# JARVIS-MoCap/JARVIS-HybridNet

Measured on AMD Instinct MI355X. Metric: multi-view frames/s (12cam 1280x1024, 23kpt, 64^3 grid), higher is better.
Workload: dtype f32; 1 GPU; BASELINE configs[2]: HybridNet 12-camera 1280x1024, 23 kpts, 64^3 grid, small/small; cameras=12, joints=23, grid=64, streams=3, parallelism=single GPU, 3 time batches in flight on 3 HIP streams, hipgraph=False

## Files before the change

### include/jarvis_hip.h

```cpp
#ifndef JARVIS_HIP_H
#define JARVIS_HIP_H
#include <stdint.h>

#ifdef __cplusplus
extern "C" {
#endif

#define JH_ABI_VERSION 4

const char* jh_last_error(void);
int jh_abi_version(void);

#define JH_PRECISION_DEFAULT (-1)
#define JH_PRECISION_F32 0
#define JH_PRECISION_BF16X3 1
#define JH_PRECISION_BF16X3_WIDE 2
int jh_set_precision(int mode);
int jh_get_precision(void);

typedef struct jh_params jh_params;
int jh_params_create(jh_params** out);
int jh_params_set(jh_params* p, const char* key, const float* host, int64_t numel);
void jh_params_destroy(jh_params* p);

// ... 258 lines not shown
int jh_predictor2d_forward_sensor(jh_predictor2d* pr, const uint8_t* frames_dev, const jh_sensor_surface* surface,
                                  int32_t* points_dev, float* conf_dev, int32_t* valid_dev, void* stream);

int jh_predictor2d_forward_images(jh_predictor2d* pr, const void* const* images_host, int n_images, int format,
                                  const jh_yuv_surface* yuv, const jh_sensor_surface* sensor,
                                  int32_t* points_dev, float* conf_dev, int32_t* valid_dev, void* stream);

int jh_profile_begin(void);
int jh_profile_end(int* n_records);
int jh_profile_get(int i, char* name, int name_cap, double* ms, double* flops, double* bytes);

int jh_op_conv(int nd, int kind, int k, int stride, int pad, int cin, int cout,
               const float* w_host, const float* b_host, const float* x_dev, int n, int d, int h,
               int w, const float* gate_dev, int norm_act, float* y_dev, void* stream);
long jh_deconv4_window_launches(void);
int jh_conv_form(int nd, int kind, int k, int stride, int pad, int cin, int cout, int has_bias,
                 int want_stats, int gate , int precision,
                 int in_px , char* name, int name_cap);
int jh_node_form(int c, int cout, int n, int h, int w, int n_in, const int* modes, int act, int batch_class,
                 int want_pool, char* name, int name_cap, int32_t out[8]);
typedef struct jh_op_operand {
  const double* in_sums_host;
  int32_t in_act;
  int32_t latency_class;
  int32_t want_stats;
  int32_t se_c, se_s;
  float se_inv_hw;
  const float *se_wr_host, *se_br_host, *se_we_host, *se_be_host;
  const double* se_pool_host;
} jh_op_operand;
int jh_op_conv_operand(int nd, int kind, int k, int stride, int pad, int cin, int cout,
                       const float* w_host, const float* b_host, const float* x_dev, int n, int d, int h,
                       int w, const float* gate_dev, const jh_op_operand* operand, float* y_dev, void* stream);
int jh_op_se_gate(const double* pool_host, int n, int c, int squeeze, float inv_hw, const float* wr_host,
                  const float* br_host, const float* we_host, const float* be_host, float* gate_dev, void* stream);
int jh_op_norm_apply(const float* x_dev, int n, int c, int d, int h, int w, const double* sums_host, int act,
                     const float* r1_dev, const double* r1_sums_host, const float* r2_dev, int write_y, int want_pool,
                     int min_block_kb, float* y_dev, double* pool_host, void* stream);
int jh_op_depthwise(int k, int c, const float* w_host, const float* x_dev, int n, int h, int w,
                    int norm_act, float* y_dev, void* stream);
int jh_op_depthwise_pool(int k, int c, const float* w_host, const float* x_dev, int n, int h, int w,
                         float* y_dev, float* pool_dev, void* stream);

int jh_op_yuv420_to_bgr(const uint8_t* frames_dev, int format, int n, int h, int w, uint8_t* out_bgr_dev,
                        void* stream);
int jh_op_yuv_surface_to_bgr(const uint8_t* frames_dev, const jh_yuv_surface* surface, int n, int h, int w,
                             uint8_t* out_bgr_dev, void* stream);
int jh_op_sensor_to_bgr(const uint8_t* frames_dev, const jh_sensor_surface* surface, int n, int h, int w,
                        uint8_t* out_bgr_dev, void* stream);

int64_t jh_joint_argmax_all_workspace_bytes(int n, int hh, int wh, int jp);
int jh_op_joint_argmax_all(const float* heat_dev, int n, int hh, int wh, int j, int jp, int32_t* idx_dev,
                           float* max_dev, void* workspace_dev, int64_t workspace_bytes, void* stream);

int jh_op_bifpn_node(int n_in, const int* modes, const float* weights, int act, int n, int c, int cout,
                     int h, int w, const float* x0_dev, const float* x1_dev, const float* x2_dev,
                     const float* dw_host, const float* pw_host, const float* bias_host, float* y_dev,
                     void* stream);
typedef struct jh_op_node_ex {
  int32_t batch_class;
  int32_t want_pool;
  const double* in_sums_host[3];
  int64_t in_count[3];
  float* y_pool_dev;
  int32_t* pool_written_host;
  double* out_sums_host;
// ... 11 lines not shown
```

### jarvis-hybridnet_amd/_native.py

```python
import ctypes
import math
import os
from typing import NamedTuple

import torch

_HERE = os.path.dirname(os.path.abspath(__file__))
LIB_PATH = os.environ.get("JH_LIBRARY_PATH") or os.path.join(_HERE, "libjarvis_hip.so")
_lib = None

c_void_p, c_int, c_float, c_int64 = ctypes.c_void_p, ctypes.c_int, ctypes.c_float, ctypes.c_int64
c_char_p = ctypes.c_char_p


class PredictorConfig(ctypes.Structure):
    _fields_ = [("num_cameras", ctypes.c_int32), ("num_joints", ctypes.c_int32),
                ("center_size", ctypes.c_int32), ("bbox", ctypes.c_int32),
                ("roi_cube_size", c_float), ("grid_spacing", c_float),
                ("center_model", ctypes.c_int32), ("kp_model", ctypes.c_int32),
                ("img_h", ctypes.c_int32), ("img_w", ctypes.c_int32),
                ("time_batch", ctypes.c_int32), ("time_batch_3d", ctypes.c_int32),
                ("cam_lo", ctypes.c_int32),
                ("cam_n", ctypes.c_int32), ("mean", c_float * 3), ("std", c_float * 3),
                ("precision", ctypes.c_int32)]
# ... 185 lines not shown
    "jh_op_joint_peaks_refine": (c_int, [c_void_p, c_int, c_int, c_int, c_int, c_void_p, c_int, c_int, c_void_p,
                                         c_void_p]),
    "jh_op_triangulate_joints": (c_int, [c_void_p, c_int, c_int, c_int, c_void_p, c_void_p, c_void_p, c_int,
                                         ctypes.POINTER(Joints3dParamsStruct), c_void_p, c_void_p, c_void_p, c_void_p,
                                         c_void_p]),
    "jh_predictor_triangulate_joints": (c_int, [c_void_p, c_void_p, c_int, c_void_p,
                                                ctypes.POINTER(Joints3dParamsStruct)] + [c_void_p] * 6),
    "jh_predictor_set_joint_mask": (c_int, [c_void_p, c_int, c_void_p, ctypes.POINTER(Joints3dParamsStruct), c_void_p]),
    "jh_predictor_get_joint_mask": (c_int, [c_void_p, c_void_p, c_void_p, c_void_p]),
    "jh_predictor_stage_3d_joint_masked": (c_int, [c_void_p, c_void_p, c_int] + [c_void_p] * 6),
    "jh_reproject_joint_masked_workspace_bytes": (c_int64, [c_int, c_int, c_int, c_int]),
    "jh_reproject_forward_joint_masked": (c_int, [c_void_p, c_int, c_int, c_int, c_void_p, c_void_p, c_void_p,
                                                  c_void_p, c_void_p, c_int, c_float, c_void_p, c_void_p, c_void_p,
                                                  c_void_p, c_int64, c_void_p]),
    "jh_joint_argmax_all_workspace_bytes": (c_int64, [c_int, c_int, c_int, c_int]),
    "jh_op_joint_argmax_all": (c_int, [c_void_p, c_int, c_int, c_int, c_int, c_int, c_void_p, c_void_p, c_void_p,
                                       c_int64, c_void_p]),
    "jh_predictor2d_create": (c_int, [c_void_p, c_void_p, ctypes.POINTER(PredictorConfig),
                                      ctypes.POINTER(c_void_p)]),
    "jh_predictor2d_destroy": (None, [c_void_p]),
    "jh_predictor2d_forward": (c_int, [c_void_p] * 6),
    "jh_predictor2d_forward_u8": (c_int, [c_void_p] * 6),
    "jh_predictor2d_forward_yuv": (c_int, [c_void_p, c_void_p, c_int, c_void_p, c_void_p, c_void_p, c_void_p]),
    "jh_predictor_debug": (c_int, [c_void_p, c_void_p, c_void_p, c_void_p, c_void_p, c_void_p]),
    "jh_predictor_hybridnet_forward": (c_int, [c_void_p] * 9),
    "jh_op_conv": (c_int, [c_int] * 7 + [c_void_p, c_void_p, c_void_p] + [c_int] * 4 +
                   [c_void_p, c_int, c_void_p, c_void_p]),
    "jh_deconv4_window_launches": (ctypes.c_long, []),
    "jh_conv_form": (c_int, [c_int] * 12 + [c_char_p, c_int]),
    "jh_node_form": (c_int, [c_int] * 6 + [ctypes.POINTER(c_int)] + [c_int] * 3 +
                     [c_char_p, c_int, ctypes.POINTER(ctypes.c_int32)]),
    "jh_op_conv_operand": (c_int, [c_int] * 7 + [c_void_p, c_void_p, c_void_p] + [c_int] * 4 +
                           [c_void_p, ctypes.POINTER(OpOperand), c_void_p, c_void_p]),
    "jh_op_se_gate": (c_int, [c_void_p, c_int, c_int, c_int, c_float] + [c_void_p] * 6),
    "jh_op_norm_apply": (c_int, [c_void_p] + [c_int] * 5 + [c_void_p, c_int, c_void_p, c_void_p, c_void_p, c_int,
                                                           c_int, c_int, c_void_p, c_void_p, c_void_p]),
    "jh_op_depthwise": (c_int, [c_int, c_int, c_void_p, c_void_p, c_int, c_int, c_int, c_int,
                                c_void_p, c_void_p]),
    "jh_op_depthwise_pool": (c_int, [c_int, c_int, c_void_p, c_void_p, c_int, c_int, c_int, c_void_p, c_void_p,
                                     c_void_p]),
    "jh_op_yuv420_to_bgr": (c_int, [c_void_p, c_int, c_int, c_int, c_int, c_void_p, c_void_p]),
    "jh_op_bifpn_node": (c_int, [c_int, ctypes.POINTER(c_int), ctypes.POINTER(c_float), c_int, c_int, c_int,
                                 c_int, c_int, c_int, c_void_p, c_void_p, c_void_p, c_void_p, c_void_p,
                                 c_void_p, c_void_p, c_void_p]),
    "jh_op_bifpn_node_ex": (c_int, [c_int, ctypes.POINTER(c_int), ctypes.POINTER(c_float), c_int, c_int, c_int,
                                    c_int, c_int, c_int, c_void_p, c_void_p, c_void_p, c_void_p, c_void_p,
                                    c_void_p, c_void_p, ctypes.POINTER(OpNodeEx), c_void_p]),
}


def symbols():
    return sorted(_SIGS)


def lib():
    global _lib
    if _lib is None:
        if not os.path.isfile(LIB_PATH):
            raise RuntimeError(
                "jarvis_hybridnet_amd: %s is missing -- build it with "
                "`python -c 'import __graft_entry__ as g; g.build()'` (hipcc, gfx950). "
                "There is no CPU fallback." % LIB_PATH)
        handle = ctypes.CDLL(LIB_PATH)
        for name, (res, args) in _SIGS.items():
            fn = getattr(handle, name)
            fn.restype, fn.argtypes = res, args
# ... 398 lines not shown
```

### jarvis-hybridnet_amd/csrc/api.hip

```cpp
#include <cstring>
#include <memory>
#include "../../include/jarvis_hip.h"
#include <cstdlib>
#include "nets.h"
#include "bifpn_node.h"
#include "views2d.h"
#include "subjects.h"
#include "joints3d.h"
#include "tracks.h"

namespace jh {
static thread_local std::string g_err;
void set_error(const std::string& msg) { g_err = msg; }
}

using namespace jh;

struct jh_params { ParamMap map; };
struct jh_efftrack { EffTrackPlan plan; };
struct jh_v2v { V2VPlan plan; };

namespace {

struct Scratch {
// ... 1683 lines not shown
                        (int32_t)ch.lds, ch.pool ? 1 : 0};
  std::copy(v, v + 8, out);
  return 0;
}

static int op_upload_stats(Scratch& sc, const double* sums_host, int n, int c, int Cp, double** dev) {
  std::vector<double> st((size_t)n * Cp * kStatW, 0.0);
  for (int b = 0; b < n; ++b)
    for (int ch = 0; ch < c; ++ch) {
      st[((size_t)b * Cp + ch) * kStatW] = sums_host[((size_t)b * c + ch) * 2];
      st[((size_t)b * Cp + ch) * kStatW + kLimbs] = sums_host[((size_t)b * c + ch) * 2 + 1];
    }
  return op_upload(sc, st.data(), st.size(), dev);
}

static int op_upload_se(Scratch& sc, const double* pool_host, int n, int C, int Cp, int S, float inv_hw,
                        const float* wr, const float* br, const float* we, const float* be, SeGate* out) {
  JH_REQUIRE(pool_host && wr && br && we && be && C >= 1 && C <= Cp && S >= 1, "squeeze-excite recipe");
  std::vector<double> pl((size_t)n * Cp * kLimbs, 0.0);
  for (int b = 0; b < n; ++b)
    for (int ch = 0; ch < C; ++ch) pl[((size_t)b * Cp + ch) * kLimbs] = pool_host[(size_t)b * C + ch];
  double* pool = nullptr;
  float *dwr = nullptr, *dbr = nullptr, *dwe = nullptr, *dbe = nullptr;
  if (op_upload(sc, pl.data(), pl.size(), &pool) || op_upload(sc, wr, (size_t)S * C, &dwr) ||
      op_upload(sc, br, (size_t)S, &dbr) || op_upload(sc, we, (size_t)C * S, &dwe) || op_upload(sc, be, (size_t)C, &dbe))
    return 1;
  out->pool = pool; out->wr = dwr; out->br = dbr; out->we = dwe; out->be = dbe;
  out->C = C; out->S = S; out->inv_hw = inv_hw;
  return 0;
}

static int op_conv_body(int nd, int kind, int k, int stride, int pad, int cin, int cout, const float* w_host,
                        const float* b_host, const float* x_dev, int n, int d, int h, int w, const float* gate_dev,
                        int norm_act, const jh_op_operand* opd, float* y_dev, hipStream_t s, const char* who) {
  const bool recipe = opd && opd->se_pool_host;
  const bool want_stats = opd ? opd->want_stats != 0 : norm_act >= 0;
  const bool plain_out = !want_stats && !gate_dev && !recipe;
  const ConvDesc desc = kind == 0 ? conv_desc(nd, k, stride, pad, cin, cout)
                                  : (kind == 1 ? deconv2d_k4s2p1_desc(cin, cout) : deconv3d_k2s2_desc(cin, cout));
  Scratch sc;
  Act x, y;
  if (nd == 2) d = 1;
  if (sc.act(n, d, h, w, cin, &x)) return 1;
  int Do, Ho, Wo;
  conv_out_shape(desc, d, h, w, &Do, &Ho, &Wo);
  if (sc.act(n, Do, Ho, Wo, cout, &y)) return 1;
  JH_CHECK_HIP(hipMemsetAsync(y.p, kind == 1 && plain_out ? 0xFF : 0, y.bytes(), s));
  ConvUse use;
  use.desc = desc; use.desc.latency_class = opd ? opd->latency_class : 0;
  use.transposed = kind != 0; use.has_bias = b_host != nullptr; use.want_stats = want_stats;
  use.gate = recipe ? ConvGate::Recipe : (gate_dev ? ConvGate::Tensor : ConvGate::None);
  use.precision = precision_mode();
  use.in_px = x.Cp;
  ConvLayer layer;
  if (make_conv_layer(use, w_host, b_host, y.D, y.H, y.W, &layer)) return 1;
  double* stats = nullptr;
  float* gate_p = nullptr;
  if (want_stats) {
    if (sc.get(reinterpret_cast<void**>(&stats), (size_t)n * y.Cp * kStatW * sizeof(double))) return 1;
    JH_CHECK_HIP(hipMemsetAsync(stats, 0, (size_t)n * y.Cp * kStatW * sizeof(double), s));
  }
  if (gate_dev) {
    if (sc.get(reinterpret_cast<void**>(&gate_p), (size_t)n * x.Cp * sizeof(float))) return 1;
    JH_CHECK_HIP(hipMemsetAsync(gate_p, 0, (size_t)n * x.Cp * sizeof(float), s));
    JH_CHECK_HIP(hipMemcpy2DAsync(gate_p, x.Cp * sizeof(float), gate_dev, cin * sizeof(float), cin * sizeof(float), n,
                                  hipMemcpyDeviceToDevice, s));
  }
  InNorm in;
  SeGate se;
  if (opd && opd->in_sums_host) {
    double* st = nullptr;
    if (op_upload_stats(sc, opd->in_sums_host, n, cin, x.Cp, &st)) return 1;
    in.stats = st; in.inv = 1.f / (float)x.pixels(); in.act = opd->in_act;
  }
  if (recipe) {
    JH_REQUIRE(opd->se_c == cin, "the gate recipe has one gate per input channel");
    if (op_upload_se(sc, opd->se_pool_host, n, opd->se_c, x.Cp, opd->se_s, opd->se_inv_hw, opd->se_wr_host,
                     opd->se_br_host, opd->se_we_host, opd->se_be_host, &se)) return 1;
  }
  if (launch_to_channel_last(x_dev, x, s)) return 1;
  if (layer.launch(x, y, gate_p, stats, in, recipe ? &se : nullptr, s)) return 1;
  if (!opd && norm_act >= 0 && launch_norm_apply(y, stats, norm_act, nullptr, nullptr, y.p, nullptr, s)) return 1;
  if (launch_from_channel_last(y, y_dev, s)) return 1;
  if (hipStreamSynchronize(s) != hipSuccess) { set_error(std::string("stream sync failed in ") + who); return 1; }
  return 0;
}

int jh_op_conv(int nd, int kind, int k, int stride, int pad, int cin, int cout,
               const float* w_host, const float* b_host, const float* x_dev, int n, int d, int h,
               int w, const float* gate_dev, int norm_act, float* y_dev, void* stream) {
  return op_conv_body(nd, kind, k, stride, pad, cin, cout, w_host, b_host, x_dev, n, d, h, w, gate_dev, norm_act,
                      nullptr, y_dev, static_cast<hipStream_t>(stream), "jh_op_conv");
}

int jh_op_conv_operand(int nd, int kind, int k, int stride, int pad, int cin, int cout,
                       const float* w_host, const float* b_host, const float* x_dev, int n, int d, int h,
                       int w, const float* gate_dev, const jh_op_operand* operand, float* y_dev, void* stream) {
  JH_REQUIRE(operand && w_host && x_dev && y_dev && n >= 1, "bad argument");
  JH_REQUIRE(operand->in_act >= ACT_NONE && operand->in_act <= ACT_SILU, "jh_op_conv_operand: in_act");
  JH_REQUIRE(operand->latency_class == 0 || operand->latency_class == 1, "jh_op_conv_operand: latency_class");
  JH_REQUIRE(!(gate_dev && operand->se_pool_host), "either a gate tensor or a gate recipe");
  return op_conv_body(nd, kind, k, stride, pad, cin, cout, w_host, b_host, x_dev, n, d, h, w, gate_dev, -1, operand,
                      y_dev, static_cast<hipStream_t>(stream), "jh_op_conv_operand");
}

int jh_op_se_gate(const double* pool_host, int n, int c, int squeeze, float inv_hw, const float* wr_host,
                  const float* br_host, const float* we_host, const float* be_host, float* gate_dev, void* stream) {
  hipStream_t s = static_cast<hipStream_t>(stream);
  JH_REQUIRE(gate_dev && n >= 1, "bad argument");
  Scratch sc;
  SeGate se;
  const int Cp = cpad(c);
  if (op_upload_se(sc, pool_host, n, c, Cp, squeeze, inv_hw, wr_host, br_host, we_host, be_host, &se)) return 1;
  float* gate = nullptr;
  if (sc.get(reinterpret_cast<void**>(&gate), (size_t)n * Cp * sizeof(float))) return 1;
  if (launch_se_gate(se.pool, n, c, Cp, squeeze, inv_hw, se.wr, se.br, se.we, se.be, gate, s)) return 1;
  JH_CHECK_HIP(hipMemcpy2DAsync(gate_dev, c * sizeof(float), gate, Cp * sizeof(float), c * sizeof(float), n,
                                hipMemcpyDeviceToDevice, s));
  JH_CHECK_HIP(hipStreamSynchronize(s));
  return 0;
}

int jh_op_norm_apply(const float* x_dev, int n, int c, int d, int h, int w, const double* sums_host, int act,
                     const float* r1_dev, const double* r1_sums_host, const float* r2_dev, int write_y, int want_pool,
                     int min_block_kb, float* y_dev, double* pool_host, void* stream) {
  hipStream_t s = static_cast<hipStream_t>(stream);
  JH_REQUIRE(x_dev && sums_host && n >= 1 && (!write_y || y_dev) && (!want_pool || pool_host), "bad argument");
  Scratch sc;
  Act x, r1, r2;
  if (sc.act(n, d, h, w, c, &x) || launch_to_channel_last(x_dev, x, s)) return 1;
  if (r1_dev && (sc.act(n, d, h, w, c, &r1) || launch_to_channel_last(r1_dev, r1, s))) return 1;
  if (r2_dev && (sc.act(n, d, h, w, c, &r2) || launch_to_channel_last(r2_dev, r2, s))) return 1;
  double *st = nullptr, *st1 = nullptr, *pool = nullptr;
  if (op_upload_stats(sc, sums_host, n, c, x.Cp, &st)) return 1;
  if (r1_sums_host && op_upload_stats(sc, r1_sums_host, n, c, x.Cp, &st1)) return 1;
  const size_t npl = (size_t)n * x.Cp * kLimbs;
// ... 259 lines not shown
```

### jarvis-hybridnet_amd/csrc/conv3d_wino.hip

```cpp
#include <vector>
#include "conv_mfma.h"
#include "conv3d_wino.h"

namespace jh {

constexpr int kWSV = 12;

constexpr int kWTZ = 4;
template <int NR, bool SH = false>
__global__ __launch_bounds__(256, 1) void conv3d_wino_kernel(const WinoArgs a) {
  constexpr int kWPZ = kWTZ + 2;
  constexpr int kWNP = kWPZ * (SH ? 108 : kWPY * kWPX);
  extern __shared__ __attribute__((aligned(16))) float lds_all[];
  const int nrm_floats = a.in_stats ? 2 * a.cin_p : 0;
  float* nrm = lds_all;
  float* R = lds_all + nrm_floats;
  float* V = R + kWNP * 8;
  float* X = R;
  const int tid = threadIdx.x;
  const int lane = tid & 63;
  const int wave = __builtin_amdgcn_readfirstlane(tid >> 6);
  const int mrow = lane & 15, kq = lane >> 4;

  const BlockId bid = xcd_block();
// ... 213 lines not shown
        X[(wave * NR * 16 + nr * 16 + mrow) * 2 + 1] = t2;
      }
    }
    __syncthreads();
    if (tid < NR * 16) {
      const int ch = nb0 * 16 + tid;
      if (ch < a.cout_p) {
        float t1 = 0.f, t2 = 0.f;
#pragma unroll
        for (int w = 0; w < 4; ++w) {
          t1 += X[(w * NR * 16 + tid) * 2 + 0];
          t2 += X[(w * NR * 16 + tid) * 2 + 1];
        }
        stat_add(a.stats + ((size_t)n * a.cout_p + ch) * kStatW, t1, t2);
      }
    }
  }
}

template <int NR, bool SH = false>
static int launch_wino_nr(const WinoArgs& a, dim3 grid, size_t lds, hipStream_t s) {
  auto kern = conv3d_wino_kernel<NR, SH>;
  static bool big = false;
  if (!big) {
    JH_CHECK_HIP(hipFuncSetAttribute(reinterpret_cast<const void*>(kern),
                                     hipFuncAttributeMaxDynamicSharedMemorySize, 160 * 1024));
    big = true;
  }
  hipLaunchKernelGGL(kern, grid, dim3(256), lds, s, a);
  JH_CHECK_HIP(hipGetLastError());
  return 0;
}

int pack_wino_weights(int cin, int cout, const float* w, const float* b, ConvWeights* out) {
  const int cin_p = cpad(cin), cout_p16 = round_up(cout, 16);
  const int nk8 = cin_p / 8, nb = cout_p16 / 16;
  static const float G[4][3] = {{1.f, 0.f, 0.f}, {.5f, .5f, .5f}, {.5f, -.5f, .5f}, {0.f, 0.f, 1.f}};
  std::vector<float> packed((size_t)16 * 3 * nk8 * nb * 128, 0.f);
  for (int co = 0; co < cout; ++co)
    for (int ci = 0; ci < cin; ++ci)
      for (int dz = 0; dz < 3; ++dz) {
        const float* g = w + (((size_t)co * cin + ci) * 3 + dz) * 9;
        double tmp[4][3];
        for (int fy = 0; fy < 4; ++fy)
          for (int kx = 0; kx < 3; ++kx) {
            double s = 0.0;
            for (int ky = 0; ky < 3; ++ky) s += (double)G[fy][ky] * g[ky * 3 + kx];
            tmp[fy][kx] = s;
          }
        const int k8 = ci / 8, kq = (ci % 8) / 2, j = ci % 2;
        const int nbk = co / 16, nn = co % 16;
        const int lane = kq * 16 + nn;
        for (int fy = 0; fy < 4; ++fy)
          for (int fx = 0; fx < 4; ++fx) {
            double s = 0.0;
            for (int kx = 0; kx < 3; ++kx) s += tmp[fy][kx] * (double)G[fx][kx];
            const int f = fy * 4 + fx;
            packed[((((size_t)f * 3 + dz) * nk8 + k8) * nb + nbk) * 128 + lane * 2 + j] = (float)s;
          }
      }
  out->cin_p = cin_p; out->cout_p16 = cout_p16; out->phase_stride = packed.size();
  return upload_conv_weights(packed.data(), packed.size() * sizeof(float), b, cout, out);
}

std::vector<int> wino_tables(int D, int H, int W, int cin_p) {
  const WinoTiling g = wino_tiling(D, H, W, 4);
  std::vector<int> t;
  if (!g.shaped) return t;
  t.assign((size_t)3 * kWinoShapeWords, 0);
  const int rz = D % 4 ? D % 4 : 4;
  for (int lc = 1; lc <= 3; ++lc) {
    const int PW = (2 << lc) + 2, PH = (32 >> lc) + 2, TH = 32 >> lc, TW = 2 << lc;
    const int hy = H - (lc == 3 ? g.H44 : 0), wx = W - (lc == 1 ? g.W44 : 0);
    const int ry = hy % TH ? hy % TH : TH, rx = wx % TW ? wx % TW : TW;
    int* tab = t.data() + (size_t)(lc - 1) * kWinoShapeWords;
    for (int lane = 0; lane < 64; ++lane) {
      unsigned m[7] = {0, 0, 0, 0, 0, 0, 0};
      for (int it = 0; it < kWinoShapeIter; ++it) {
        const int idx = lane + it * 64, pix = idx >> 1, q = lane & 1;
        const int px = pix % PW, py = (pix / PW) % PH, pz = pix / (PW * PH);
        tab[it * 64 + lane] = (((pz * H + py) * W + px) * cin_p + q * 4) * 4;
        m[0] |= (unsigned)(pz == 0) << it; m[1] |= (unsigned)(pz > rz) << it;
        m[2] |= (unsigned)(py == 0) << it; m[3] |= (unsigned)(py > ry) << it;
        m[4] |= (unsigned)(px == 0) << it; m[5] |= (unsigned)(px > rx) << it;
        m[6] |= (unsigned)(idx >= 6 * PW * PH * 2) << it;
      }
      for (int k = 0; k < 7; ++k) tab[(kWinoShapeIter + k) * 64 + lane] = (int)m[k];
    }
  }
  return t;
}
// ... 39 lines not shown
```

### jarvis-hybridnet_amd/csrc/conv_layer.h

```cpp
#pragma once
#include <string>
#include <vector>
#include "jh_common.h"

namespace jh {

enum class ConvForm {
  Mfma,
  Wino,
  WinoBf16x3,
  ConvBf16x3,
  Deconv4Bf16x3,
  DeconvC1,
};

enum class ConvGate { None = 0, Tensor = 1, Recipe = 2 };

struct ConvUse {
  ConvDesc desc;
  bool transposed = false;
  bool has_bias = false;
  bool want_stats = false;
  ConvGate gate = ConvGate::None;
  int precision = 0;
  int in_px = 0;
};

struct ConvChoice {
  ConvForm form = ConvForm::Mfma;
  WeightLayout layout = WeightLayout::Plain;
  int wino_variant = 0;
};
ConvChoice choose_conv(const ConvUse& u);
std::string conv_choice_name(const ConvChoice& c);

std::vector<float> taps_major(const float* w, int channels, int taps, int Cp);

struct ConvLayer {
  ConvLayer() = default;
  ConvLayer(const ConvLayer&) = delete;
  ConvLayer& operator=(const ConvLayer&) = delete;
  ~ConvLayer();

  ConvChoice choice;
  ConvDesc desc{};
  ConvWeights w;
  int* wino_tiles = nullptr;
  size_t table_bytes = 0;

  int launch(const Act& x, const Act& y, const float* gate, double* stats, const InNorm& in, const SeGate* se,
             hipStream_t s) const;
  std::string profile_name(int out_w) const;
  size_t device_bytes() const { return w.phase_stride * desc.nphase * sizeof(float) + table_bytes; }
};

int make_conv_layer(const ConvUse& u, const float* w_host, const float* b_host, int D, int H, int W, ConvLayer* out);

}
// ... 1 lines not shown
```

### jarvis-hybridnet_amd/csrc/conv_layer.hip

```cpp
#include <cstdlib>
#include "conv_layer.h"
#include "conv_mfma.h"
#include "conv3d_wino.h"

namespace jh {

static int knob_now(const char* name, int unset) {
  const char* e = getenv(name);
  return e ? atoi(e) : unset;
}

static WeightLayout conv_weight_layout(const ConvUse& u) {
  const ConvDesc& d = u.desc;
  const int cin_p = cpad(d.cin), cout_p = cpad(d.cout), cout_p16 = round_up(d.cout, 16);
  if (d.nd == 3 && d.k == 3 && d.stride == 2 && d.ostride == 1) return WeightLayout::TapPaired;
  if (d.nd == 2 && d.ostride > 1) {
    const int wmode = knob_now("JH_DECONV4_WINDOW", 1);
    if (!u.want_stats && u.gate == ConvGate::None && wmode != 0 && deconv4_window_eligible(cin_p, cout_p, wmode >= 2))
      return WeightLayout::Window;
    if (deconv4_eligible(cin_p, cout_p16)) return WeightLayout::ChannelPaired;
  }
  return WeightLayout::Plain;
}

ConvChoice choose_conv(const ConvUse& u) {
  const ConvDesc& d = u.desc;
  const bool ungated = u.gate == ConvGate::None;
  const bool bare_deconv2d = d.nd == 2 && d.ostride > 1 && u.transposed && !u.has_bias && !u.want_stats && ungated;
  const int in_px = u.in_px ? u.in_px : cpad(d.cin);
  const auto form = [](ConvForm f, int wino_variant = 0) { return ConvChoice{f, WeightLayout::Plain, wino_variant}; };
  if (bare_deconv2d && d.cout == 1) return form(ConvForm::DeconvC1);
  if (d.nd == 3 && d.k == 3 && d.stride == 1 && d.ostride == 1 && d.phase[0].pad[2] == 1 && !u.transposed && ungated &&
      knob_now("JH_WINO", 1) != 0)
    return form(u.precision >= 1 ? ConvForm::WinoBf16x3 : ConvForm::Wino, knob_now("JH_WINO_PW", 1) != 0 ? 4 : 0);
  if (bare_deconv2d && u.precision >= 1 && deconv4_bf16x3_eligible(d.cout)) return form(ConvForm::Deconv4Bf16x3);
  if (!u.transposed && ungated && conv_bf16x3_eligible(d) && in_px == cpad(d.cin) &&
      (u.precision == 2 || (u.precision == 1 && d.nd == 3)))
    return form(ConvForm::ConvBf16x3);
  return ConvChoice{ConvForm::Mfma, conv_weight_layout(u), 0};
}

std::string conv_choice_name(const ConvChoice& c) {
  static const char* const forms[] = {"mfma", "wino", "wino_bf16x3", "conv_bf16x3", "deconv4_bf16x3", "deconv_c1"};
  static const char* const layouts[] = {"", "_paired", "_tappair", "_window"};
  return std::string(forms[(int)c.form]) + (c.form == ConvForm::Mfma ? layouts[(int)c.layout] : "");
}

std::vector<float> taps_major(const float* w, int channels, int taps, int Cp) {
  std::vector<float> wt((size_t)taps * Cp, 0.f);
  for (int c = 0; c < channels; ++c)
    for (int t = 0; t < taps; ++t) wt[(size_t)t * Cp + c] = w[(size_t)c * taps + t];
  return wt;
}

ConvLayer::~ConvLayer() {
  free_conv_weights(&w);
  if (wino_tiles) (void)hipFree(wino_tiles);
}

int make_conv_layer(const ConvUse& u, const float* w_host, const float* b_host, int D, int H, int W, ConvLayer* out) {
  const ConvDesc& d = u.desc;
  JH_REQUIRE(w_host && (b_host != nullptr) == u.has_bias, "conv layer weights / bias");
  const ConvChoice c = out->choice = choose_conv(u);
  const int in_px = u.in_px ? u.in_px : cpad(d.cin);
  out->desc = d;
  switch (c.form) {
    case ConvForm::DeconvC1: {
      const std::vector<float> wt = taps_major(w_host, d.cin, 16, in_px);
      out->w.phase_stride = wt.size() / d.nphase;
      return upload_conv_weights(wt.data(), wt.size() * sizeof(float), nullptr, 0, &out->w);
    }
    case ConvForm::ConvBf16x3: return pack_conv_bf16x3_weights(d, w_host, b_host, &out->w);
    case ConvForm::Deconv4Bf16x3: return pack_deconv4_bf16x3_weights(d.cin, d.cout, w_host, &out->w);
    case ConvForm::WinoBf16x3: return pack_bf16x3_weights(d.cin, d.cout, w_host, b_host, &out->w);
    case ConvForm::Mfma: return pack_conv_weights(d, w_host, b_host, u.transposed, c.layout, &out->w);
    case ConvForm::Wino: break;
  }
  if (pack_wino_weights(d.cin, d.cout, w_host, b_host, &out->w)) return 1;
  const std::vector<int> tt = wino_tables(D, H, W, in_px);
  if (tt.empty()) return 0;
  out->table_bytes = tt.size() * sizeof(int);
  JH_CHECK_HIP(hipMalloc(&out->wino_tiles, out->table_bytes));
  JH_CHECK_HIP(hipMemcpy(out->wino_tiles, tt.data(), out->table_bytes, hipMemcpyHostToDevice));
  return 0;
}

int ConvLayer::launch(const Act& x, const Act& y, const float* gate, double* stats, const InNorm& in, const SeGate* se,
                      hipStream_t s) const {
  JH_REQUIRE(choice.form == ConvForm::Mfma || (!gate && !(se && se->pool)), "only the MFMA form takes a gate");
  switch (choice.form) {
    case ConvForm::DeconvC1: return launch_deconv_c1(x, in.stats, in.inv, in.act, w.w, y, s);
    case ConvForm::ConvBf16x3: return launch_conv_bf16x3(desc, w, x, y, stats, s, &in);
    case ConvForm::Deconv4Bf16x3: return launch_deconv4_bf16x3(w, x, y, s, &in);
    case ConvForm::WinoBf16x3: return launch_conv3d_bf16x3(w, x, y, stats, s, &in);
    case ConvForm::Wino: return launch_conv3d_wino(w, x, y, stats, s, &in, choice.wino_variant, wino_tiles);
    case ConvForm::Mfma: return launch_conv(desc, w, x, y, gate, stats, s, &in, se);
  }
  JH_REQUIRE(false, "conv form");
}

std::string ConvLayer::profile_name(int out_w) const {
  if (choice.form == ConvForm::DeconvC1) return "deconv_k4s2T_c1";
  const ConvDesc& d = desc;
  const bool up = d.ostride > 1;
  const bool split = choice.form == ConvForm::WinoBf16x3 || choice.form == ConvForm::ConvBf16x3;
  const char* tag = up ? (choice.form == ConvForm::Deconv4Bf16x3 ? "Tbf16x3" : "T")
                       : (split ? "bf16x3" : (choice.form == ConvForm::Wino ? "wino" : ""));
  char nm[96];
  snprintf(nm, sizeof nm, "conv%dd_k%ds%d%s_%dx%d@%d", d.nd, up ? (d.nd == 2 ? 4 : 2) : d.k, up ? 2 : d.stride, tag,
           d.cin, d.cout, out_w);
  return nm;
}

}
```

### jarvis-hybridnet_amd/csrc/jh_common.h

```cpp
#pragma once
#include <hip/hip_runtime.h>
#include <cstdlib>
#include <cstdint>
#include <cstdio>
#include <cstring>
#include <string>
#include <vector>

namespace jh {

constexpr int kWave = 64;

#define JH_ENV_KNOB(name) ([]() -> int { static const int v = [] { const char* e = getenv(name); return e ? atoi(e) : -1; }(); return v; }())

inline int round_up(int v, int m) { return (v + m - 1) / m * m; }
inline int cpad(int c) { return round_up(c, 8); }

void set_error(const std::string& msg);
#define JH_CHECK_HIP(expr)                                                     \
  do {                                                                         \
    hipError_t _e = (expr);                                                    \
    if (_e != hipSuccess) {                                                    \
      jh::set_error(std::string(#expr) + ": " + hipGetErrorString(_e));        \
      return 1;                                                                \
// ... 233 lines not shown
  unsigned l = xcd_linear(L, gx * gy * gz);
  BlockId b;
  b.x = l % gx; l /= gx;
  b.y = l % gy;
  b.z = l / gy;
  return b;
}
#endif

#if defined(__HIPCC__)
__device__ __forceinline__ float sum_xor16(float s) {
  const auto r = __builtin_amdgcn_permlane16_swap(__float_as_uint(s), __float_as_uint(s), false, false);
  return __uint_as_float(r[0]) + __uint_as_float(r[1]);
}
__device__ __forceinline__ float sum_xor32(float s) {
  const auto r = __builtin_amdgcn_permlane32_swap(__float_as_uint(s), __float_as_uint(s), false, false);
  return __uint_as_float(r[0]) + __uint_as_float(r[1]);
}
__device__ __forceinline__ double sum_xor16(double s) {
  const unsigned lo = (unsigned)__double2loint(s), hi = (unsigned)__double2hiint(s);
  const auto a = __builtin_amdgcn_permlane16_swap(lo, lo, false, false);
  const auto b = __builtin_amdgcn_permlane16_swap(hi, hi, false, false);
  return __hiloint2double((int)b[0], (int)a[0]) + __hiloint2double((int)b[1], (int)a[1]);
}
__device__ __forceinline__ double sum_xor32(double s) {
  const unsigned lo = (unsigned)__double2loint(s), hi = (unsigned)__double2hiint(s);
  const auto a = __builtin_amdgcn_permlane32_swap(lo, lo, false, false);
  const auto b = __builtin_amdgcn_permlane32_swap(hi, hi, false, false);
  return __hiloint2double((int)b[0], (int)a[0]) + __hiloint2double((int)b[1], (int)a[1]);
}
__device__ __forceinline__ float silu_fast(float v) { return v * __builtin_amdgcn_rcpf(1.f + __expf(-v)); }
#endif

int pack_wino_weights(int cin, int cout, const float* w, const float* b, ConvWeights* out);
int launch_conv3d_wino(const ConvWeights& w, const Act& x, const Act& y, double* stats, hipStream_t s,
                       const InNorm* in, int variant, const int* tables);
bool v2v_fold_shape(int J, int G);
bool v2v_fold_applies(int J, int G);
int launch_conv3d_out_fold(const ConvWeights& w, const Act& r_dec, const double* st_dec, const float* u0,
                           const double* st_u0, const float* r_skip, const double* st_skip, const float* f1,
                           const Act& y, hipStream_t s);
inline unsigned short bf16_rne(float f) {
  unsigned u;
  std::memcpy(&u, &f, 4);
  u += 0x7fffu + ((u >> 16) & 1u);
  return (unsigned short)(u >> 16);
}
inline float bf16_to_f32(unsigned short h) {
  const unsigned u = (unsigned)h << 16;
  float f;
  std::memcpy(&f, &u, 4);
  return f;
}
int pack_bf16x3_weights(int cin, int cout, const float* w, const float* b, ConvWeights* out);
int launch_conv3d_bf16x3(const ConvWeights& w, const Act& x, const Act& y, double* stats, hipStream_t s,
                         const InNorm* in);
int pack_deconv4_bf16x3_weights(int cin, int cout, const float* w, ConvWeights* out);
bool deconv4_bf16x3_eligible(int cout);
int launch_deconv4_bf16x3(const ConvWeights& w, const Act& x, const Act& y, hipStream_t s, const InNorm* in);
bool conv_bf16x3_eligible(const ConvDesc& d);
int pack_conv_bf16x3_weights(const ConvDesc& d, const float* w, const float* b, ConvWeights* out);
int launch_conv_bf16x3(const ConvDesc& d, const ConvWeights& w, const Act& x, const Act& y, double* stats,
                       hipStream_t s, const InNorm* in);
int precision_mode();
void set_precision_mode(int m);
void pack_stem_weights(const float* w_host, float* packed, int cout);
int launch_stem_conv(const Act& x, const float* w_dev, const Act& y, double* stats, hipStream_t s);
struct StemSource;
int launch_stem_conv_src(const StemSource& src, const Act& x, const float* w_dev, const Act& y, double* stats,
// ... 11 lines not shown
```

Measured before the change: 2180 multi-view frames/s.

## Add Winograd F(2x2,3x3) MFMA kernel for 2D 3x3 stride-1 convolutions

```diff
diff --git a/include/jarvis_hip.h b/include/jarvis_hip.h
--- a/include/jarvis_hip.h
+++ b/include/jarvis_hip.h
@@ -314,6 +314,10 @@
 int jh_op_conv_operand(int nd, int kind, int k, int stride, int pad, int cin, int cout,
                        const float* w_host, const float* b_host, const float* x_dev, int n, int d, int h,
                        int w, const float* gate_dev, const jh_op_operand* operand, float* y_dev, void* stream);
+int jh_op_conv_operand_sums(int nd, int kind, int k, int stride, int pad, int cin, int cout,
+                            const float* w_host, const float* b_host, const float* x_dev, int n, int d, int h,
+                            int w, const float* gate_dev, const jh_op_operand* operand, float* y_dev,
+                            double* out_sums_host, void* stream);
 int jh_op_se_gate(const double* pool_host, int n, int c, int squeeze, float inv_hw, const float* wr_host,
                   const float* br_host, const float* we_host, const float* be_host, float* gate_dev, void* stream);
 int jh_op_norm_apply(const float* x_dev, int n, int c, int d, int h, int w, const double* sums_host, int act,
diff --git a/jarvis-hybridnet_amd/_native.py b/jarvis-hybridnet_amd/_native.py
--- a/jarvis-hybridnet_amd/_native.py
+++ b/jarvis-hybridnet_amd/_native.py
@@ -241,6 +241,8 @@
                      [c_char_p, c_int, ctypes.POINTER(ctypes.c_int32)]),
     "jh_op_conv_operand": (c_int, [c_int] * 7 + [c_void_p, c_void_p, c_void_p] + [c_int] * 4 +
                            [c_void_p, ctypes.POINTER(OpOperand), c_void_p, c_void_p]),
+    "jh_op_conv_operand_sums": (c_int, [c_int] * 7 + [c_void_p, c_void_p, c_void_p] + [c_int] * 4 +
+                                [c_void_p, ctypes.POINTER(OpOperand), c_void_p, c_void_p, c_void_p]),
     "jh_op_se_gate": (c_int, [c_void_p, c_int, c_int, c_int, c_float] + [c_void_p] * 6),
     "jh_op_norm_apply": (c_int, [c_void_p] + [c_int] * 5 + [c_void_p, c_int, c_void_p, c_void_p, c_void_p, c_int,
                                                            c_int, c_int, c_void_p, c_void_p, c_void_p]),
diff --git a/jarvis-hybridnet_amd/csrc/api.hip b/jarvis-hybridnet_amd/csrc/api.hip
--- a/jarvis-hybridnet_amd/csrc/api.hip
+++ b/jarvis-hybridnet_amd/csrc/api.hip
@@ -1739,7 +1739,8 @@
 
 static int op_conv_body(int nd, int kind, int k, int stride, int pad, int cin, int cout, const float* w_host,
                         const float* b_host, const float* x_dev, int n, int d, int h, int w, const float* gate_dev,
-                        int norm_act, const jh_op_operand* opd, float* y_dev, hipStream_t s, const char* who) {
+                        int norm_act, const jh_op_operand* opd, float* y_dev, hipStream_t s, const char* who,
+                        double* out_sums_host = nullptr) {
   const bool recipe = opd && opd->se_pool_host;
   const bool want_stats = opd ? opd->want_stats != 0 : norm_act >= 0;
   const bool plain_out = !want_stats && !gate_dev && !recipe;
@@ -1789,7 +1790,16 @@
   if (layer.launch(x, y, gate_p, stats, in, recipe ? &se : nullptr, s)) return 1;
   if (!opd && norm_act >= 0 && launch_norm_apply(y, stats, norm_act, nullptr, nullptr, y.p, nullptr, s)) return 1;
   if (launch_from_channel_last(y, y_dev, s)) return 1;
+  std::vector<double> hst(out_sums_host && stats ? (size_t)n * y.Cp * kStatW : 0);
+  if (!hst.empty())
+    JH_CHECK_HIP(hipMemcpyAsync(hst.data(), stats, hst.size() * sizeof(double), hipMemcpyDeviceToHost, s));
   if (hipStreamSynchronize(s) != hipSuccess) { set_error(std::string("stream sync failed in ") + who); return 1; }
+  for (int b = 0; b < n && !hst.empty(); ++b)
+    for (int ch = 0; ch < cout; ++ch) {
+      const double* q = hst.data() + ((size_t)b * y.Cp + ch) * kStatW;
+      out_sums_host[((size_t)b * cout + ch) * 2] = (q[0] + q[1]) + q[2];
+      out_sums_host[((size_t)b * cout + ch) * 2 + 1] = (q[kLimbs] + q[kLimbs + 1]) + q[kLimbs + 2];
+    }
   return 0;
 }
 
@@ -1809,6 +1819,19 @@
   JH_REQUIRE(!(gate_dev && operand->se_pool_host), "either a gate tensor or a gate recipe");
   return op_conv_body(nd, kind, k, stride, pad, cin, cout, w_host, b_host, x_dev, n, d, h, w, gate_dev, -1, operand,
                       y_dev, static_cast<hipStream_t>(stream), "jh_op_conv_operand");
+}
+
+int jh_op_conv_operand_sums(int nd, int kind, int k, int stride, int pad, int cin, int cout,
+                            const float* w_host, const float* b_host, const float* x_dev, int n, int d, int h,
+                            int w, const float* gate_dev, const jh_op_operand* operand, float* y_dev,
+                            double* out_sums_host, void* stream) {
+  JH_REQUIRE(operand && w_host && x_dev && y_dev && out_sums_host && n >= 1, "bad argument");
+  JH_REQUIRE(operand->want_stats != 0, "jh_op_conv_operand_sums: the launch must accumulate statistics");
+  JH_REQUIRE(operand->in_act >= ACT_NONE && operand->in_act <= ACT_SILU, "jh_op_conv_operand_sums: in_act");
+  JH_REQUIRE(operand->latency_class == 0 || operand->latency_class == 1, "jh_op_conv_operand_sums: latency_class");
+  JH_REQUIRE(!(gate_dev && operand->se_pool_host), "either a gate tensor or a gate recipe");
+  return op_conv_body(nd, kind, k, stride, pad, cin, cout, w_host, b_host, x_dev, n, d, h, w, gate_dev, -1, operand,
+                      y_dev, static_cast<hipStream_t>(stream), "jh_op_conv_operand_sums", out_sums_host);
 }
 
 int jh_op_se_gate(const double* pool_host, int n, int c, int squeeze, float inv_hw, const float* wr_host,
diff --git a/jarvis-hybridnet_amd/csrc/conv2d_wino.hip b/jarvis-hybridnet_amd/csrc/conv2d_wino.hip
--- /dev/null
+++ b/jarvis-hybridnet_amd/csrc/conv2d_wino.hip
@@ -0,0 +1,232 @@
+#include <algorithm>
+#include "conv_mfma.h"
+#include "conv3d_wino.h"
+
+namespace jh {
+
+constexpr int kWSV = 12;
+constexpr int k2PW = 18;
+constexpr int k2NP = k2PW * k2PW;
+constexpr int k2VF = 4 * 16 * 16 * kWSV;
+constexpr int k2XC = 4 * 64 + 16;
+constexpr int k2LoopFloats = k2NP * 8 + k2VF;
+constexpr int wino2d_x_floats(int nr) { return 4 * 2 * 4 * nr * k2XC; }
+constexpr int wino2d_red_at(int nr) {
+  return wino2d_x_floats(nr) > k2LoopFloats ? wino2d_x_floats(nr) : k2LoopFloats;
+}
+
+template <int NR>
+__global__ __launch_bounds__(256, NR == 1 ? 2 : 1) void conv2d_wino_kernel(const WinoArgs a) {
+  extern __shared__ __attribute__((aligned(16))) float lds_all[];
+  const int nrm_floats = a.in_stats ? 2 * a.cin_p : 0;
+  float* nrm = lds_all;
+  float* R = lds_all + nrm_floats;
+  float* V = R + k2NP * 8;
+  float* X = R;
+  float* red = R + wino2d_red_at(NR);
+  const int tid = threadIdx.x;
+  const int lane = tid & 63;
+  const int wave = __builtin_amdgcn_readfirstlane(tid >> 6);
+  const int mrow = lane & 15, kq = lane >> 4;
+
+  const BlockId bid = xcd_block();
+  const int bx_n = (a.W + 15) / 16;
+  const int x0 = ((int)bid.x % bx_n) * 16, y0 = ((int)bid.x / bx_n) * 16;
+  const int nb0 = bid.y * NR;
+  const int n = bid.z;
+  const int nk8 = a.cin_p >> 3, nb = a.cout_p16 >> 4;
+
+  if (a.in_stats) norm_table_fill(NormTable::FmaRstd, nrm, a.cin_p, a.in_stats, n, a.cin_p, a.in_inv, tid, 256);
+  const float* __restrict__ xin = a.x + (size_t)n * a.H * a.W * a.cin_p;
+
+  f32x4 acc[4][4][NR];
+#pragma unroll
+  for (int fi = 0; fi < 4; ++fi)
+#pragma unroll
+    for (int mr = 0; mr < 4; ++mr)
+#pragma unroll
+      for (int nr = 0; nr < NR; ++nr) acc[fi][mr][nr] = (f32x4){0.f, 0.f, 0.f, 0.f};
+
+  constexpr int ITER = (k2NP * 2 + 255) / 256;
+  float4 pf[ITER];
+  int poff[ITER];
+  unsigned okmask = 0;
+#pragma unroll
+  for (int it = 0; it < ITER; ++it) {
+    const int idx = tid + it * 256;
+    const int q = idx & 1, pix = idx >> 1;
+    const int px = pix % k2PW, py = pix / k2PW;
+    const int iy = y0 - 1 + py, ix = x0 - 1 + px;
+    const bool ok = idx < k2NP * 2 && iy >= 0 && iy < a.H && ix >= 0 && ix < a.W;
+    poff[it] = ok ? (iy * a.W + ix) * a.cin_p + q * 4 : 0;
+    okmask |= ok ? (1u << it) : 0u;
+  }
+#pragma unroll
+  for (int it = 0; it < ITER; ++it)
+    pf[it] = (okmask >> it & 1) ? *reinterpret_cast<const float4*>(xin + poff[it]) : make_float4(0.f, 0.f, 0.f, 0.f);
+
+  const float2* __restrict__ U2 = reinterpret_cast<const float2*>(a.u);
+  const float2* V2 = reinterpret_cast<const float2*>(V);
+  int boff[NR];
+#pragma unroll
+  for (int nr = 0; nr < NR; ++nr) boff[nr] = min(nb0 + nr, nb - 1) * 64 + lane;
+
+  const int cp = tid & 3, tm = (tid >> 2) & 15;
+  const int tty = 2 * wave + (tm >> 3), ttx = tm & 7;
+  const float* rb = R + ((2 * tty) * k2PW + 2 * ttx) * 8 + cp * 2;
+  float* vb = V + ((wave * 16) * 16 + tm) * kWSV + cp * 2;
+
+  for (int c0 = 0; c0 < a.cin_p; c0 += 8) {
+    float2 b0v[NR];
+#pragma unroll
+    for (int nr = 0; nr < NR; ++nr) b0v[nr] = U2[(size_t)(((wave * 4) * nk8 + (c0 >> 3)) * nb) * 64 + boff[nr]];
+    __syncthreads();
+#pragma unroll
+    for (int it = 0; it < ITER; ++it) {
+      const int idx = tid + it * 256;
+      if (idx < k2NP * 2) {
+        float4 v = pf[it];
+        if ((okmask >> it & 1) && a.in_stats) {
+          const int c = c0 + (idx & 1) * 4;
+          const float4 nm = *reinterpret_cast<const float4*>(nrm + c);
+          const float4 rs = *reinterpret_cast<const float4*>(nrm + a.cin_p + c);
+          v = act4(norm_fma4(v, nm, rs), a.in_act);
+        }
+        *reinterpret_cast<float4*>(R + idx * 4) = v;
+      }
+    }
+    __syncthreads();
+    if (c0 + 8 < a.cin_p) {
+#pragma unroll
+      for (int it = 0; it < ITER; ++it)
+        pf[it] = (okmask >> it & 1) ? *reinterpret_cast<const float4*>(xin + poff[it] + c0 + 8)
+                                    : make_float4(0.f, 0.f, 0.f, 0.f);
+    }
+    {
+      float2 tr[4][4];
+#pragma unroll
+      for (int r = 0; r < 4; ++r) {
+        const float2 d0 = *reinterpret_cast<const float2*>(rb + (r * k2PW + 0) * 8);
+        const float2 d1 = *reinterpret_cast<const float2*>(rb + (r * k2PW + 1) * 8);
+        const float2 d2 = *reinterpret_cast<const float2*>(rb + (r * k2PW + 2) * 8);
+        const float2 d3 = *reinterpret_cast<const float2*>(rb + (r * k2PW + 3) * 8);
+        tr[r][0] = make_float2(d0.x - d2.x, d0.y - d2.y);
+        tr[r][1] = make_float2(d1.x + d2.x, d1.y + d2.y);
+        tr[r][2] = make_float2(d2.x - d1.x, d2.y - d1.y);
+        tr[r][3] = make_float2(d1.x - d3.x, d1.y - d3.y);
+      }
+#pragma unroll
+      for (int fx = 0; fx < 4; ++fx) {
+        const float2 t0 = tr[0][fx], t1 = tr[1][fx], t2 = tr[2][fx], t3 = tr[3][fx];
+        *reinterpret_cast<float2*>(vb + (0 * 4 + fx) * 16 * kWSV) = make_float2(t0.x - t2.x, t0.y - t2.y);
+        *reinterpret_cast<float2*>(vb + (1 * 4 + fx) * 16 * kWSV) = make_float2(t1.x + t2.x, t1.y + t2.y);
+        *reinterpret_cast<float2*>(vb + (2 * 4 + fx) * 16 * kWSV) = make_float2(t2.x - t1.x, t2.y - t1.y);
+        *reinterpret_cast<float2*>(vb + (3 * 4 + fx) * 16 * kWSV) = make_float2(t1.x - t3.x, t1.y - t3.y);
+      }
+    }
+    __syncthreads();
+    const int kk = c0 >> 3;
+#pragma unroll
+    for (int fi = 0; fi < 4; ++fi) {
+      const int f = wave * 4 + fi;
+      float2 av[4], bv[NR];
+#pragma unroll
+      for (int mr = 0; mr < 4; ++mr) av[mr] = V2[((mr * 16 + f) * 16 + mrow) * (kWSV / 2) + kq];
+#pragma unroll
+      for (int nr = 0; nr < NR; ++nr)
+        bv[nr] = fi == 0 ? b0v[nr] : U2[(size_t)((f * nk8 + kk) * nb) * 64 + boff[nr]];
+#pragma unroll
+      for (int mr = 0; mr < 4; ++mr)
+#pragma unroll
+        for (int nr = 0; nr < NR; ++nr)
+          acc[fi][mr][nr] = __builtin_amdgcn_mfma_f32_16x16x4f32(av[mr].x, bv[nr].x, acc[fi][mr][nr], 0, 0, 0);
+#pragma unroll
+      for (int mr = 0; mr < 4; ++mr)
+#pragma unroll
+        for (int nr = 0; nr < NR; ++nr)
+          acc[fi][mr][nr] = __builtin_amdgcn_mfma_f32_16x16x4f32(av[mr].y, bv[nr].y, acc[fi][mr][nr], 0, 0, 0);
+    }
+  }
+
+  __syncthreads();
+#pragma unroll
+  for (int mr = 0; mr < 4; ++mr)
+#pragma unroll
+    for (int nr = 0; nr < NR; ++nr) {
+      const f32x4 m0 = acc[0][mr][nr], m1 = acc[1][mr][nr], m2 = acc[2][mr][nr], m3 = acc[3][mr][nr];
+      float* xa = X + (((wave * 2 + 0) * 4 + mr) * NR + nr) * k2XC + lane;
+      float* xb = X + (((wave * 2 + 1) * 4 + mr) * NR + nr) * k2XC + lane;
+#pragma unroll
+      for (int r = 0; r < 4; ++r) {
+        xa[r * 64 + (r >> 1) * 16] = m0[r] + m1[r] + m2[r];
+        xb[r * 64 + (r >> 1) * 16] = m1[r] - m2[r] - m3[r];
+      }
+    }
+  __syncthreads();
+  f32x4 out[4][NR];
+#pragma unroll
+  for (int nr = 0; nr < NR; ++nr)
+#pragma unroll
+    for (int th = 0; th < 2; ++th)
+#pragma unroll
+      for (int r = 0; r < 4; ++r) {
+        const int sk = 2 * th + (kq >> 1), sr = 2 * (kq & 1) + (r >> 1);
+        const int at = sr * 64 + (sr >> 1) * 16 + sk * 16 + mrow;
+        float p[4];
+#pragma unroll
+        for (int w = 0; w < 4; ++w) p[w] = X[(((w * 2 + (r & 1)) * 4 + wave) * NR + nr) * k2XC + at];
+        out[2 * th + 0][nr][r] = p[0] + p[1] + p[2];
+        out[2 * th + 1][nr][r] = p[1] - p[2] - p[3];
+      }
+
+  EpilogueArgs e;
+  e.y = a.y + (size_t)n * a.H * a.W * a.cout_p;
+  e.bias = a.bias;
+  e.stats = a.stats ? a.stats + (size_t)n * a.cout_p * kStatW : nullptr;
+  e.Dout = 1; e.Hout = a.H; e.Wout = a.W; e.Hy = a.H; e.Wy = a.W;
+  e.cout_p = a.cout_p; e.cout_p16 = a.cout_p16; e.os = 1; e.osz = 1;
+  e.offz = 0; e.offy = 0; e.offx = 0;
+  if (y0 + 16 <= a.H && x0 + 16 <= a.W)
+    conv_epilogue<4, NR, 16, 16, 4, true>(out, e, red, nb0, 0, y0, x0, tid);
+  else
+    conv_epilogue<4, NR, 16, 16>(out, e, red, nb0, 0, y0, x0, tid);
+}
+
+template <int NR>
+static int launch_wino2d_nr(const WinoArgs& a, dim3 grid, size_t lds, hipStream_t s) {
+  auto kern = conv2d_wino_kernel<NR>;
+  static bool big = false;
+  if (!big) {
+    JH_CHECK_HIP(hipFuncSetAttribute(reinterpret_cast<const void*>(kern),
+                                     hipFuncAttributeMaxDynamicSharedMemorySize, 160 * 1024));
+    big = true;
+  }
+  hipLaunchKernelGGL(kern, grid, dim3(256), lds, s, a);
+  JH_CHECK_HIP(hipGetLastError());
+  return 0;
+}
+
+int launch_conv2d_wino(const ConvWeights& w, const Act& x, const Act& y, double* stats, hipStream_t s,
+                       const InNorm* in) {
+  JH_REQUIRE(x.Cp == w.cin_p && x.N == y.N && x.D == 1 && y.D == 1 && x.H == y.H && x.W == y.W, "wino2d shapes");
+  JH_REQUIRE(y.Cp <= w.cout_p16 && (long)x.H * x.W * std::max(x.Cp, y.Cp) < (1L << 31) && x.N <= 65535, "wino2d extent");
+  WinoArgs a{};
+  a.x = x.p; a.y = y.p; a.u = w.w; a.bias = w.bias; a.stats = stats;
+  if (in && in->stats) { a.in_stats = in->stats; a.in_inv = in->inv; a.in_act = in->act; }
+  a.N = x.N; a.D = 1; a.H = x.H; a.W = x.W; a.cin_p = x.Cp; a.cout_p = y.Cp; a.cout_p16 = w.cout_p16;
+  const int nb = w.cout_p16 / 16;
+  const int blocks = ((x.H + 15) / 16) * ((x.W + 15) / 16);
+  int nr = (nb % 3 == 0) ? 3 : ((nb % 2 == 0) ? 2 : (nb == 1 ? 1 : 3));
+  while (nr > 1 && (long)blocks * ((nb + nr - 1) / nr) * x.N <= 128) --nr;
+  dim3 grid(blocks, (nb + nr - 1) / nr, x.N);
+  const size_t lds = ((size_t)wino2d_red_at(nr) + (a.in_stats ? (size_t)2 * a.cin_p : 0)) * sizeof(float) +
+                     (size_t)4 * nr * 16 * 2 * sizeof(double);
+  JH_REQUIRE(lds <= 160 * 1024, "wino2d LDS");
+#define JH_WINO2D_CASE(NRV) \
+  if (nr == NRV) return launch_wino2d_nr<NRV>(a, grid, lds, s);
+  JH_WINO2D_CASE(3) JH_WINO2D_CASE(2) JH_WINO2D_CASE(1)
+#undef JH_WINO2D_CASE
+  JH_REQUIRE(false, "wino2d NR");
+}
+
+}
diff --git a/jarvis-hybridnet_amd/csrc/conv3d_wino.hip b/jarvis-hybridnet_amd/csrc/conv3d_wino.hip
--- a/jarvis-hybridnet_amd/csrc/conv3d_wino.hip
+++ b/jarvis-hybridnet_amd/csrc/conv3d_wino.hip
@@ -269,15 +269,15 @@
   return 0;
 }
 
-int pack_wino_weights(int cin, int cout, const float* w, const float* b, ConvWeights* out) {
+int pack_wino_weights(int cin, int cout, int nz, const float* w, const float* b, ConvWeights* out) {
   const int cin_p = cpad(cin), cout_p16 = round_up(cout, 16);
   const int nk8 = cin_p / 8, nb = cout_p16 / 16;
   static const float G[4][3] = {{1.f, 0.f, 0.f}, {.5f, .5f, .5f}, {.5f, -.5f, .5f}, {0.f, 0.f, 1.f}};
-  std::vector<float> packed((size_t)16 * 3 * nk8 * nb * 128, 0.f);
+  std::vector<float> packed((size_t)16 * nz * nk8 * nb * 128, 0.f);
   for (int co = 0; co < cout; ++co)
     for (int ci = 0; ci < cin; ++ci)
-      for (int dz = 0; dz < 3; ++dz) {
-        const float* g = w + (((size_t)co * cin + ci) * 3 + dz) * 9;
+      for (int dz = 0; dz < nz; ++dz) {
+        const float* g = w + (((size_t)co * cin + ci) * nz + dz) * 9;
         double tmp[4][3];
         for (int fy = 0; fy < 4; ++fy)
           for (int kx = 0; kx < 3; ++kx) {
@@ -293,7 +293,7 @@
             double s = 0.0;
             for (int kx = 0; kx < 3; ++kx) s += tmp[fy][kx] * (double)G[fx][kx];
             const int f = fy * 4 + fx;
-            packed[((((size_t)f * 3 + dz) * nk8 + k8) * nb + nbk) * 128 + lane * 2 + j] = (float)s;
+            packed[((((size_t)f * nz + dz) * nk8 + k8) * nb + nbk) * 128 + lane * 2 + j] = (float)s;
           }
       }
   out->cin_p = cin_p; out->cout_p16 = cout_p16; out->phase_stride = packed.size();
diff --git a/jarvis-hybridnet_amd/csrc/conv_layer.h b/jarvis-hybridnet_amd/csrc/conv_layer.h
--- a/jarvis-hybridnet_amd/csrc/conv_layer.h
+++ b/jarvis-hybridnet_amd/csrc/conv_layer.h
@@ -12,6 +12,7 @@
   ConvBf16x3,
   Deconv4Bf16x3,
   DeconvC1,
+  Wino2d,
 };
 
 enum class ConvGate { None = 0, Tensor = 1, Recipe = 2 };
@@ -24,6 +25,7 @@
   ConvGate gate = ConvGate::None;
   int precision = 0;
   int in_px = 0;
+  int out_h = 0, out_w = 0;
 };
 
 struct ConvChoice {
diff --git a/jarvis-hybridnet_amd/csrc/conv_layer.hip b/jarvis-hybridnet_amd/csrc/conv_layer.hip
--- a/jarvis-hybridnet_amd/csrc/conv_layer.hip
+++ b/jarvis-hybridnet_amd/csrc/conv_layer.hip
@@ -9,6 +9,8 @@
   const char* e = getenv(name);
   return e ? atoi(e) : unset;
 }
+
+constexpr int kWino2dMinCin = 40;
 
 static WeightLayout conv_weight_layout(const ConvUse& u) {
   const ConvDesc& d = u.desc;
@@ -37,11 +39,18 @@
   if (!u.transposed && ungated && conv_bf16x3_eligible(d) && in_px == cpad(d.cin) &&
       (u.precision == 2 || (u.precision == 1 && d.nd == 3)))
     return form(ConvForm::ConvBf16x3);
+  const int wino2d = knob_now("JH_WINO2D", 1);
+  if (d.nd == 2 && d.k == 3 && d.stride == 1 && d.ostride == 1 && d.nphase == 1 && d.phase[0].pad[1] == 1 &&
+      d.phase[0].pad[2] == 1 && !u.transposed && ungated && in_px == cpad(d.cin) && in_px >= 16 && wino2d != 0) {
+    const long regions = (long)((u.out_h + 15) / 16) * ((u.out_w + 15) / 16);
+    const bool filled = u.out_h <= 0 || u.out_w <= 0 || 8L * u.out_h * u.out_w >= 7L * 256 * regions;
+    if (wino2d >= 2 || (in_px >= kWino2dMinCin && filled)) return form(ConvForm::Wino2d);
+  }
   return ConvChoice{ConvForm::Mfma, conv_weight_layout(u), 0};
 }
 
 std::string conv_choice_name(const ConvChoice& c) {
-  static const char* const forms[] = {"mfma", "wino", "wino_bf16x3", "conv_bf16x3", "deconv4_bf16x3", "deconv_c1"};
+  static const char* const forms[] = {"mfma", "wino", "wino_bf16x3", "conv_bf16x3", "deconv4_bf16x3", "deconv_c1", "wino2d"};
   static const char* const layouts[] = {"", "_paired", "_tappair", "_window"};
   return std::string(forms[(int)c.form]) + (c.form == ConvForm::Mfma ? layouts[(int)c.layout] : "");
 }
@@ -61,7 +70,9 @@
 int make_conv_layer(const ConvUse& u, const float* w_host, const float* b_host, int D, int H, int W, ConvLayer* out) {
   const ConvDesc& d = u.desc;
   JH_REQUIRE(w_host && (b_host != nullptr) == u.has_bias, "conv layer weights / bias");
-  const ConvChoice c = out->choice = choose_conv(u);
+  ConvUse placed = u;
+  placed.out_h = H; placed.out_w = W;
+  const ConvChoice c = out->choice = choose_conv(placed);
   const int in_px = u.in_px ? u.in_px : cpad(d.cin);
   out->desc = d;
   switch (c.form) {
@@ -74,9 +85,10 @@
     case ConvForm::Deconv4Bf16x3: return pack_deconv4_bf16x3_weights(d.cin, d.cout, w_host, &out->w);
     case ConvForm::WinoBf16x3: return pack_bf16x3_weights(d.cin, d.cout, w_host, b_host, &out->w);
     case ConvForm::Mfma: return pack_conv_weights(d, w_host, b_host, u.transposed, c.layout, &out->w);
+    case ConvForm::Wino2d: return pack_wino_weights(d.cin, d.cout, 1, w_host, b_host, &out->w);
     case ConvForm::Wino: break;
   }
-  if (pack_wino_weights(d.cin, d.cout, w_host, b_host, &out->w)) return 1;
+  if (pack_wino_weights(d.cin, d.cout, 3, w_host, b_host, &out->w)) return 1;
   const std::vector<int> tt = wino_tables(D, H, W, in_px);
   if (tt.empty()) return 0;
   out->table_bytes = tt.size() * sizeof(int);
@@ -94,6 +106,7 @@
     case ConvForm::Deconv4Bf16x3: return launch_deconv4_bf16x3(w, x, y, s, &in);
     case ConvForm::WinoBf16x3: return launch_conv3d_bf16x3(w, x, y, stats, s, &in);
     case ConvForm::Wino: return launch_conv3d_wino(w, x, y, stats, s, &in, choice.wino_variant, wino_tiles);
+    case ConvForm::Wino2d: return launch_conv2d_wino(w, x, y, stats, s, &in);
     case ConvForm::Mfma: return launch_conv(desc, w, x, y, gate, stats, s, &in, se);
   }
   JH_REQUIRE(false, "conv form");
@@ -105,7 +118,7 @@
   const bool up = d.ostride > 1;
   const bool split = choice.form == ConvForm::WinoBf16x3 || choice.form == ConvForm::ConvBf16x3;
   const char* tag = up ? (choice.form == ConvForm::Deconv4Bf16x3 ? "Tbf16x3" : "T")
-                       : (split ? "bf16x3" : (choice.form == ConvForm::Wino ? "wino" : ""));
+                       : (split ? "bf16x3" : (choice.form == ConvForm::Wino || choice.form == ConvForm::Wino2d ? "wino" : ""));
   char nm[96];
   snprintf(nm, sizeof nm, "conv%dd_k%ds%d%s_%dx%d@%d", d.nd, up ? (d.nd == 2 ? 4 : 2) : d.k, up ? 2 : d.stride, tag,
            d.cin, d.cout, out_w);
diff --git a/jarvis-hybridnet_amd/csrc/jh_common.h b/jarvis-hybridnet_amd/csrc/jh_common.h
--- a/jarvis-hybridnet_amd/csrc/jh_common.h
+++ b/jarvis-hybridnet_amd/csrc/jh_common.h
@@ -289,9 +289,11 @@
 __device__ __forceinline__ float silu_fast(float v) { return v * __builtin_amdgcn_rcpf(1.f + __expf(-v)); }
 #endif
 
-int pack_wino_weights(int cin, int cout, const float* w, const float* b, ConvWeights* out);
+int pack_wino_weights(int cin, int cout, int nz, const float* w, const float* b, ConvWeights* out);
 int launch_conv3d_wino(const ConvWeights& w, const Act& x, const Act& y, double* stats, hipStream_t s,
                        const InNorm* in, int variant, const int* tables);
+int launch_conv2d_wino(const ConvWeights& w, const Act& x, const Act& y, double* stats, hipStream_t s,
+                       const InNorm* in);
 bool v2v_fold_shape(int J, int G);
 bool v2v_fold_applies(int J, int G);
 int launch_conv3d_out_fold(const ConvWeights& w, const Act& r_dec, const double* st_dec, const float* u0,
```

New measurement: 2162 multi-view frames/s. Within noise of the previous version (-0.8%).
